# andimarafioti/faster-qwen3-tts

Measured on AMD Instinct MI355X. Metric: real-time factor (audio s / wall s), Qwen3-TTS-12Hz-0.6B voice-clone streaming chunk_size=8; p50 TTFA in ttfa_ms_p50, higher is better.
Workload: dtype bf16

## Files before the change

faster-qwen3-tts_amd/csrc/codec_kernels.cuh:

```cuda
#pragma once
#include "fq3_common.cuh"
#include "skinny_gemm.cuh"

namespace fq3 {

typedef __attribute__((ext_vector_type(8))) __bf16 bf16x8_t;
typedef __attribute__((ext_vector_type(4))) float f32x4_t;

constexpr int kMaxTaps = 8;
struct GemmArgs {
    const void* A; int lda; int M; int a_rows;
    int m_lo;
    int n_taps; int tap_off[kMaxTaps]; int Cin;
    const void* W; int N;
    const void* bias; int bias_mod;
    const void* scale;
    const void* res; int ldr;
    void* Y; int ldy;
    int act;
    const void* sn_a; const void* sn_ib; void* Y2;
    int act2;
    float* ws; long ws_floats; int ksplit;
    int n_seg; long a_seg, y_seg, r_seg;
    int glds_min_wgs;
    int big_pair;
    const void* Wp;
    const void* Wi;
    int no_skinny;
    int glds_cap8;
    int chain;
    int glds_waves;
    int xcd_map;
    int epi_legacy;
};

// ... 583 lines not shown
#pragma unroll
            for (int j = 0; j < TN; ++j) {
                const int r = wc * (BN / WCOLS) + j * 16 + fr;
                bfr[j] = *reinterpret_cast<const bf16x8_t*>(bs + r * BK + (((ks * 4 + fq) ^ ((r >> 1) & 7)) * 8));
            }
#pragma unroll
            for (int i = 0; i < TM; ++i)
#pragma unroll
                for (int j = 0; j < TN; ++j) {
                    if constexpr (DBG == 1) { acc[i][j][0] += (float)af[i][0] + (float)bfr[j][0]; }
                    else acc[i][j] = __builtin_amdgcn_mfma_f32_16x16x32_bf16(af[i], bfr[j], acc[i][j], 0, 0, 0);
                }
        }
        buf = buf + 1 == STAGES ? 0 : buf + 1;
    }
    constexpr int kParkFloats = STAGES * (BM + BN) * BK * 2 / 4;
    if (NT == 512 || epi_can_park(a)) {
        __syncthreads();
        gemm_epilogue_parked<TE, BM, BN, TM, TN, kParkFloats, WCOLS, NT>(a, acc, m0, n0, wr, wc, lane, reinterpret_cast<float*>(glds_smem));
    } else {
        if constexpr (NT == 256) gemm_epilogue<TE, BM, BN, TM, TN>(a, acc, m0, n0, wr, wc, lane);
    }
}

template <int BN, int STAGES, typename TE = bf16_t, int NT = 256, int BM = 128, int DBG = 0>
inline void glds_go(const GemmArgs& a, hipStream_t s) {
    const int rows = a.M - a.m_lo;
    const size_t shm = (size_t)STAGES * (BM + BN) * 64 * 2;
    constexpr auto kern = glds_gemm_kernel<BN, STAGES, TE, NT, BM, DBG>;
    (void)lds_limit_at_least<kern>(shm);
    hipLaunchKernelGGL(kern, dim3((a.N + BN - 1) / BN, (rows + BM - 1) / BM, a.n_seg > 1 ? a.n_seg : 1), dim3(NT), shm, s, a);
}

template <int NW, int CH, typename TE = bf16_t>
__global__ __launch_bounds__(NW * 64) void chain_gemm_kernel(GemmArgs a_in) {
    typedef bf16_t T;
    constexpr int BM = 32, BN = 32, TM = 2, TN = 2, LDP = BN + 4, NT = NW * 64;
    __shared__ __attribute__((aligned(16))) float park[BM * LDP];
    const GemmArgs a = gemm_segment<T, TE>(a_in, (int)blockIdx.z);
    const int tid = threadIdx.x, lane = tid & 63, fr = lane & 15, fq = lane >> 4;
    const int wave = __builtin_amdgcn_readfirstlane(tid >> 6);
    const int m0 = a.m_lo + blockIdx.y * BM, n0 = blockIdx.x * BN;
    const int K = a.n_taps * a.Cin, nsteps = K / 32, nchunks = (nsteps + CH - 1) / CH;
    const T* A = reinterpret_cast<const T*>(a.A);
    const T* zero = reinterpret_cast<const T*>(g_gemm_zero_page) + fq * 8;
    int am[TM];
#pragma unroll
    for (int i = 0; i < TM; ++i) { const int m = m0 + i * 16 + fr; am[i] = m < a.M ? m : -(1 << 28); }
    const T* wrow[TN];
#pragma unroll
    for (int j = 0; j < TN; ++j) {
        int n = n0 + j * 16 + fr;
        n = n < a.N ? n : a.N - 1;
        wrow[j] = reinterpret_cast<const T*>(a.W) + (size_t)n * K + fq * 8;
    }
    u32x4 ar[CH][TM], wr[CH][TN];
    auto load_chunk = [&](int c) {
#pragma unroll
        for (int s = 0; s < CH; ++s) {
            int t = c * CH + s;
            t = t < nsteps ? t : nsteps - 1;
            const int k0 = t * 32, tap = k0 / a.Cin, ci = k0 - tap * a.Cin;
            const int toff = a_in.tap_off[tap];
#pragma unroll
            for (int i = 0; i < TM; ++i) {
                const int r = am[i] + toff;
                const T* src = (r >= 0 && r < a.a_rows) ? A + (size_t)r * a.lda + ci + fq * 8 : zero;
                ar[s][i] = *reinterpret_cast<const u32x4*>(src);
            }
#pragma unroll
            for (int j = 0; j < TN; ++j) wr[s][j] = *reinterpret_cast<const u32x4*>(wrow[j] + k0);
        }
    };
    if (wave < nchunks) load_chunk(wave);
    for (int c = 0; c < nchunks; ++c) {
        if (wave == (c % NW)) {
            f32x4_t acc[TM][TN];
#pragma unroll
            for (int i = 0; i < TM; ++i)
#pragma unroll
                for (int j = 0; j < TN; ++j)
#pragma unroll
                    for (int r = 0; r < 4; ++r) acc[i][j][r] = c ? park[(i * 16 + fq * 4 + r) * LDP + j * 16 + fr] : 0.f;
#pragma unroll
            for (int s = 0; s < CH; ++s) {
                if (c * CH + s < nsteps) {
#pragma unroll
                    for (int i = 0; i < TM; ++i)
#pragma unroll
                        for (int j = 0; j < TN; ++j)
                            acc[i][j] = __builtin_amdgcn_mfma_f32_16x16x32_bf16(__builtin_bit_cast(bf16x8_t, ar[s][i]), __builtin_bit_cast(bf16x8_t, wr[s][j]), acc[i][j], 0, 0, 0);
                }
            }
#pragma unroll
            for (int i = 0; i < TM; ++i)
#pragma unroll
                for (int j = 0; j < TN; ++j)
#pragma unroll
                    for (int r = 0; r < 4; ++r) park[(i * 16 + fq * 4 + r) * LDP + j * 16 + fr] = acc[i][j][r];
            if (c + NW < nchunks) load_chunk(c + NW);
        }
        __builtin_amdgcn_s_waitcnt(0xc07f);
        __builtin_amdgcn_s_barrier();
    }
    const EpiQ e = epiq_of(a);
    const bool quads = epi_quads_ok(a);
    for (int q = tid; q < BM * (BN / 4); q += NT) {
        const int row = q / (BN / 4), c4 = (q - row * (BN / 4)) * 4;
        const int m = m0 + row, n = n0 + c4;
        if (m >= a.M || n >= a.N) continue;
        if (quads) epi_quad<TE>(e, *reinterpret_cast<const f32x4_t*>(park + row * LDP + c4), m, n);
        else for (int cc = 0; cc < 4 && n + cc < a.N; ++cc) epilogue_elem<TE>(a, park[row * LDP + c4 + cc], m, n + cc);
    }
}
template <int NW, int CH, typename TE = bf16_t>
inline void chain_go(const GemmArgs& a, hipStream_t s) {
    const int rows = a.M - a.m_lo;
    hipLaunchKernelGGL((chain_gemm_kernel<NW, CH, TE>), dim3((a.N + 31) / 32, (rows + 31) / 32, a.n_seg > 1 ? a.n_seg : 1), dim3(NW * 64), 0, s, a);
}
inline bool chain_ok(const GemmArgs& a) {
    return a.Cin % 32 == 0 && a.act != 2 && a.ksplit <= 1 && !a.epi_legacy && a.lda % 8 == 0;
}

constexpr int kBigBM = 256, kBigBN = 256, kBigBK = 32, kBigStages = 4;
constexpr int kGldsMinWgs = 150;
template <int ST, bool TR, int BN, typename TE = bf16_t, bool PAIR = false>
__global__ __launch_bounds__(512) void big_gemm_kernel(GemmArgs a_in, int tiles_x, int tiles_seg, int tiles_total) {
    typedef bf16_t T;
    static_assert(!TR || std::is_same<TE, bf16_t>::value, "the register-layout (TR) epilogue stores bf16");
    constexpr int BM = kBigBM, BK = kBigBK, TM = 8, TN = BN / 64, WN = BN / 4, NPB = BN / 128, CP = 2 + NPB;
    static_assert(ST == 4, "ring of four stages");
    static_assert(BN == 256 || BN == 128, "256- or 128-wide tiles");
    extern __shared__ __attribute__((aligned(128))) unsigned char big_smem[];
    T* As = reinterpret_cast<T*>(big_smem);
    T* Bs = As + ST * BM * BK;
    const int tid = threadIdx.x, lane = tid & 63, fr = lane & 15, fq = lane >> 4;
    const int wave = __builtin_amdgcn_readfirstlane(tid >> 6);
    const int orig = blockIdx.x, xcd = orig & 7, q = tiles_total >> 3, r8 = tiles_total & 7;
    const int tile_all = (xcd < r8 ? xcd * (q + 1) : r8 * (q + 1) + (xcd - r8) * q) + (orig >> 3);
    const int seg = tile_all / tiles_seg, tile = tile_all - seg * tiles_seg;
    const GemmArgs a = gemm_segment<T, TE>(a_in, seg);
    const int m0 = a.m_lo + (tile / tiles_x) * BM, n0 = (tile % tiles_x) * BN;
    const int wr = wave >> 2, wc = wave & 3;
    const int K = a.n_taps * a.Cin, nsteps = K / BK;
    const T* A = reinterpret_cast<const T*>(a.A);
    const T* W = reinterpret_cast<const T*>(a.W);
    const T* zero = reinterpret_cast<const T*>(g_gemm_zero_page);
    f32x4_t acc[TM][TN];
#pragma unroll
    for (int i = 0; i < TM; ++i)
#pragma unroll
        for (int j = 0; j < TN; ++j) acc[i][j] = f32x4_t{0.f, 0.f, 0.f, 0.f};
// ... 261 lines not shown
}

template <typename T>
__global__ __launch_bounds__(256) void splitk_reduce_kernel(GemmArgs a) {
    const int rows = a.M - a.m_lo;
    const size_t e = (size_t)blockIdx.x * 256 + threadIdx.x;
    if (e >= (size_t)rows * a.N) return;
    const int mm = (int)(e / a.N), n = (int)(e % a.N), m = a.m_lo + mm;
    float sum = 0.f;
    for (int z = 0; z < a.ksplit; ++z) sum += a.ws[(size_t)z * rows * a.N + e];
    const int ch = n % a.bias_mod;
    float v = DT<T>::rnd(sum + (a.bias ? DT<T>::ld(reinterpret_cast<const T*>(a.bias) + ch) : 0.f));
    if (a.act == 1) v = DT<T>::rnd(gelu_exact(v));
    if (a.act == 3) v = DT<T>::rnd(v / (1.0f + expf(-v)));
    if (a.scale) v = DT<T>::rnd(DT<T>::ld(reinterpret_cast<const T*>(a.scale) + n) * v);
    if (a.res) v = v + DT<T>::ld(reinterpret_cast<const T*>(a.res) + (size_t)m * a.ldr + n);
    v = DT<T>::rnd(v);
    if (a.Y) DT<T>::st(reinterpret_cast<T*>(a.Y) + (size_t)m * a.ldy + n, v);
    if (a.Y2) DT<T>::st(reinterpret_cast<T*>(a.Y2) + (size_t)m * a.ldy + n,
                        snake_apply<T>(v, DT<T>::ld(reinterpret_cast<const T*>(a.sn_a) + ch), DT<T>::ld(reinterpret_cast<const T*>(a.sn_ib) + ch)));
}

template <typename T, int BM, int BN, typename TE = T>
inline void gemm_go(const GemmArgs& a, hipStream_t s) {
    constexpr int PF = (BM + BN) > 160 ? 2 : ((BM + BN) > 128 ? 4 : 8);
    dim3 grid((a.N + BN - 1) / BN, (a.M - a.m_lo + BM - 1) / BM, a.n_seg > 1 ? a.n_seg : 1);
    hipLaunchKernelGGL((conv_gemm_kernel<T, BM, BN, PF, TE>), grid, dim3(256), 0, s, a);
}
inline bool skinny_ok(const GemmArgs& a) {
    return a.ws && !a.no_skinny && a.n_taps == 1 && a.tap_off[0] == 0 && a.m_lo == 0 && a.M <= kSkinnyMaxRows && a.a_rows >= a.M && a.act == 0 &&
           !a.bias && !a.scale && !a.Y2 && a.Y && skinny_k_ok(a.Cin) && a.N % 32 == 0 && a.lda % 8 == 0 && a.ldy % 4 == 0 && (!a.res || a.ldr % 4 == 0);
}
template <typename T, typename TE>
inline void gemm_launch_te(const GemmArgs& a, hipStream_t s) {
    const int rows = a.M - a.m_lo, nseg = a.n_seg > 1 ? a.n_seg : 1;
    if (rows <= 0) return;
    if constexpr (sizeof(T) == 4) { gemm_go<T, 64, 64>(a, s); return; }
    else {
        constexpr bool kPlainBf16 = std::is_same<TE, bf16_t>::value;
        auto wgs = [&](int bm, int bn) { return (long)((rows + bm - 1) / bm) * ((a.N + bn - 1) / bn) * nseg; };
        if constexpr (kPlainBf16) {
        if (nseg == 1 && skinny_ok(a)) {
            SkinnyArgs k{};
            k.X = reinterpret_cast<const bf16_t*>(a.A); k.ldx = a.lda; k.M = a.M; k.W = reinterpret_cast<const bf16_t*>(a.W); k.N = a.N;
            k.res = reinterpret_cast<const bf16_t*>(a.res); k.ldr = a.ldr; k.Y = reinterpret_cast<bf16_t*>(a.Y); k.ldy = a.ldy;
            k.Wp = reinterpret_cast<const bf16_t*>(a.Wp);
            if (a.res) skinny_launch<SK_RESIDUAL>(k, a.Cin, s); else skinny_launch<SK_STORE>(k, a.Cin, s);
            return;
        }
        if (nseg == 1 && a.ws && a.n_taps == 1 && a.act != 2 && wgs(64, 32) < 384 && a.Cin >= 1536) {
            int S = 0;
            for (int cand : {8, 6, 4, 3, 2})
                if (a.Cin % (cand * 32) == 0 && a.Cin / (cand * 32) >= 12 && wgs(64, 32) * cand <= 1024 &&
                    (long)cand * rows * a.N <= a.ws_floats) { S = cand; break; }
            if (S > 1) {
                GemmArgs b = a;
                b.ksplit = S;
                dim3 grid((a.N + 31) / 32, (rows + 63) / 64, S);
                hipLaunchKernelGGL((conv_gemm_kernel<T, 64, 32, 8>), grid, dim3(256), 0, s, b);
                hipLaunchKernelGGL((splitk_reduce_kernel<T>), dim3((unsigned)(((size_t)rows * a.N + 255) / 256)), dim3(256), 0, s, b);
                return;
            }
        }
        }
        const bool n64 = a.N % 64 == 0 || a.N >= 512;
        if (a.act != 2 && a.Cin % 32 == 0) {
            if (big_tiling_pays(rows, a.N, kBigBN, nseg)) { big_go<TE>(a, s); return; }
            if (rows >= 1024 && a.N % 128 == 0 && big_tiling_pays(rows, a.N, 128, nseg)) {
                const bool plain = a.act == 0 && !a.scale && !a.res && !a.Y2;
                if constexpr (kPlainBf16) { if (plain) { big_go_t<true, 128>(a, s); return; } }
                big_go_t<false, 128, TE>(a, s);
                return;
            }
        }
        const long t64 = wgs(128, 64);
        const bool glds_shape = a.N % 64 == 0 && a.Cin % 64 == 0;
        const bool parks = a.act != 2 && a.ksplit <= 1 && !a.epi_legacy && a.glds_waves >= 0;
        const long t32 = wgs(32, 32);
        if (a.chain >= 0 && chain_ok(a) && t32 <= 224 && (long)a.n_taps * a.Cin >= 512 && (long)a.n_taps * a.Cin <= 4096) { chain_go<8, 8, TE>(a, s); return; }
        const long cap8 = std::is_same<TE, bfs_t>::value ? (a.glds_cap8 > 0 ? a.glds_cap8 : (1L << 30)) : 512;
        if (glds_shape && parks && t64 <= cap8 && (long)a.n_taps * a.Cin >= 512) {
            const long ta = a.N % 128 == 0 ? wgs(64, 128) : 0, tb = wgs(64, 64);
            if (ta >= 140 && ta <= cap8) glds_go<128, 3, TE, 512, 64>(a, s);
            else if (tb <= 256) glds_go<64, 3, TE, 512, 64>(a, s);
            else if (t64 <= 256) glds_go<64, 3, TE, 512>(a, s);
            else glds_go<64, 2, TE, 512>(a, s);
        } else if (glds_shape && t64 >= (a.glds_min_wgs > 0 ? a.glds_min_wgs : kGldsMinWgs)) {
            glds_go<64, 2, TE>(a, s);
        } else if (n64 && wgs(128, 64) >= 512) gemm_go<T, 128, 64, TE>(a, s);
        else if (a.act != 2 && !n64 && a.N % 96 == 0 && wgs(128, 96) >= 256) gemm_go<T, 128, 96, TE>(a, s);
        else if (a.act != 2 && !n64 && wgs(128, 32) >= 256) gemm_go<T, 128, 32, TE>(a, s);
        else if (n64 && (wgs(64, 64) >= 256 || a.act == 2)) gemm_go<T, 64, 64, TE>(a, s);
        else if (a.act == 2) gemm_go<T, 64, 64, TE>(a, s);
        else gemm_go<T, 64, 32, TE>(a, s);
    }
}
template <typename T>
inline void gemm_launch(const GemmArgs& a, hipStream_t s) {
    if constexpr (std::is_same<T, bfs_t>::value) {
        GemmArgs b = a;
        b.lda = 2 * a.lda; b.Cin = 2 * a.Cin; b.a_seg = 2 * a.a_seg;
        b.ws = nullptr;
        gemm_launch_te<bf16_t, bfs_t>(b, s);
    } else gemm_launch_te<T, T>(a, s);
}

template <typename T> __global__ void silu_mul_kernel(const T* gu, T* y, int rows, int I);

template <typename T>
inline void gemm_swiglu_halves(const GemmArgs& a, void* y, hipStream_t s) {
    const int I = a.N / 2;
    if constexpr (sizeof(T) == 2) {
        if (skinny_ok(a) && !a.res && I % 8 == 0) {
            SkinnyArgs k{};
            k.X = reinterpret_cast<const bf16_t*>(a.A); k.ldx = a.lda; k.M = a.M; k.W = reinterpret_cast<const bf16_t*>(a.W); k.N = a.N;
            k.Y = reinterpret_cast<bf16_t*>(y); k.ldy = I;
            k.Wp = reinterpret_cast<const bf16_t*>(a.Wp);
            skinny_launch<SK_SWIGLU>(k, a.Cin, s);
            return;
        }
    }
    if constexpr (std::is_same<T, bf16_t>::value) {
        const int rows = a.M - a.m_lo;
        if (a.Wi && !a.res && !a.bias && !a.scale && a.n_taps == 1 && a.N % 512 == 0 && a.Cin % 32 == 0 && a.n_seg <= 1 && I % 4 == 0 &&
            big_tiling_pays(rows, a.N, kBigBN, 1)) {
            GemmArgs b = a;
            b.W = a.Wi; b.act = 2; b.Y = y; b.ldy = I;
            big_go_t<true, kBigBN>(b, s);
            return;
        }
    }
    gemm_launch<T>(a, s);
    hipLaunchKernelGGL((silu_mul_kernel<T>), dim3((unsigned)(((size_t)a.M * I + 255) / 256)), dim3(256), 0, s, (const T*)a.Y, (T*)y, a.M, I);
}

struct RvqArgs { const void* books[32]; int nq; int n_first; int dim; };
template <typename T>
__global__ void rvq_gather_kernel(RvqArgs a, const int64_t* codes, T* first, T* rest, int Tn, int row_lo) {
// ... 210 lines not shown
```

faster-qwen3-tts_amd/csrc/fq3_codec.hip:

```cpp
#define FQ3_SKINNY_EXTERN
#include "../../include/fq3hip.h"
#include "codec_kernels.cuh"

#include <algorithm>
#include <climits>
#include <cmath>
#include <functional>
#include <map>
#include <string>
#include <vector>

using namespace fq3;

extern "C" const char* fq3_last_error(void);
extern "C" void fq3_set_error_(const char* msg);
static int cfail(int code, const std::string& m) { fq3_set_error_(m.c_str()); return code; }
#define CHIP(x) do { hipError_t e_ = (x); if (e_ != hipSuccess) return cfail(FQ3_EHIP, std::string(#x) + ": " + hipGetErrorString(e_)); } while (0)

struct fq3_codec {
    fq3_codec_config cfg{};
    int esz = 2;
    std::map<std::string, const void*> w;
    std::map<std::string, int64_t> wn;
    void* buf[4] = {nullptr, nullptr, nullptr, nullptr};
    size_t buf_elems = 0;
    void* snake_consts = nullptr;
    std::map<std::string, std::pair<const void*, const void*>> snake;
    bool ready = false;
    int glds_cap8 = 0;
    int fuse_units = 1;
};

constexpr int kPrefixOutRows = 48;
struct fq3_codec_prefix {
    fq3_codec* owner = nullptr;
    int ref_len = 0, n_pre = 0, n_kv = 0, n_out = 0;
    void *pre = nullptr, *kv = nullptr, *out = nullptr;
};

static int64_t samples_for(const fq3_codec_config& c, int64_t T) {
    int64_t n = T;
    for (int i = 0; i < c.n_upsample; ++i) n *= c.upsampling_ratios[i];
    for (int i = 0; i < c.n_rates; ++i) n = (n - 1) * c.upsample_rates[i];
    return n > 0 ? n : 0;
}

extern "C" int64_t fq3_codec_num_samples(const fq3_codec* c, int T) { return c ? samples_for(c->cfg, T) : -1; }

static size_t elems_for(const fq3_codec_config& cfg, int64_t T) {
    int64_t rows = T, mx = T * std::max(std::max(cfg.latent_dim * 4, 3 * cfg.n_heads * cfg.head_dim), cfg.decoder_dim);
    mx = std::max(mx, 2 * T * (int64_t)cfg.rvq_dim);
    for (int i = 0; i < cfg.n_upsample; ++i) { rows *= cfg.upsampling_ratios[i]; mx = std::max(mx, rows * cfg.latent_dim * 4); }
    mx = std::max(mx, rows * cfg.decoder_dim);
    int ch = cfg.decoder_dim;
    for (int i = 0; i < cfg.n_rates; ++i) { rows = (rows - 1) * cfg.upsample_rates[i]; ch /= 2; mx = std::max(mx, rows * ch); }
    return (size_t)mx + 64;
}

extern "C" int fq3_codec_create(const fq3_codec_config* cfg, fq3_codec** out) {
    if (!cfg || !out) return cfail(FQ3_EINVAL, "null argument");
    if (cfg->dtype != FQ3_BF16 && cfg->dtype != FQ3_F32 && cfg->dtype != FQ3_BF16X2) return cfail(FQ3_EINVAL, "dtype");
    if (cfg->n_upsample < 0 || cfg->n_upsample > 4 || cfg->n_rates < 1 || cfg->n_rates > 8) return cfail(FQ3_EINVAL, "upsample lists");
    if (cfg->num_quantizers > 32) return cfail(FQ3_EUNSUPPORTED, "codec dims");
    if (cfg->head_dim != 32 && cfg->head_dim != 64 && cfg->head_dim != 128) return cfail(FQ3_EUNSUPPORTED, "codec head_dim must be 32, 64 or 128");
    if (cfg->sliding_window < 1 || cfg->sliding_window > 128) return cfail(FQ3_EUNSUPPORTED, "codec sliding_window must be in 1..128");
    auto m32 = [](int v) { return v % 32 == 0; };
    int ch = cfg->decoder_dim;
    bool ok = m32(cfg->rvq_dim) && m32(cfg->codebook_dim) && m32(cfg->latent_dim) && m32(cfg->hidden) && m32(cfg->inter) &&
              m32(cfg->n_heads * cfg->head_dim) && m32(ch);
    for (int i = 0; i < cfg->n_rates; ++i) { ch /= 2; ok = ok && m32(ch); }
    if (!ok) return cfail(FQ3_EUNSUPPORTED, "every channel count must be a multiple of 32 (MFMA K step)");
    fq3_codec* c = new fq3_codec();
    c->cfg = *cfg;
    c->esz = cfg->dtype == FQ3_BF16 ? 2 : 4;
    c->buf_elems = elems_for(*cfg, cfg->max_frames);
    for (int i = 0; i < 4; ++i) {
        hipError_t e = hipMalloc(&c->buf[i], c->buf_elems * c->esz);
        if (e != hipSuccess) { for (int j = 0; j < i; ++j) (void)hipFree(c->buf[j]); delete c; return cfail(FQ3_EHIP, "hipMalloc codec workspace"); }
    }
    *out = c;
    return FQ3_OK;
}

extern "C" int fq3_codec_destroy(fq3_codec* c) {
    if (!c) return FQ3_OK;
    (void)hipDeviceSynchronize();
    for (int i = 0; i < 4; ++i) if (c->buf[i]) (void)hipFree(c->buf[i]);
    if (c->snake_consts) (void)hipFree(c->snake_consts);
    delete c;
    return FQ3_OK;
}

extern "C" int fq3_codec_set_option(fq3_codec* c, const char* key, int value) {
    if (!c || !key) return cfail(FQ3_EINVAL, "null argument");
    if (std::string(key) == "glds_cap8") c->glds_cap8 = value;
    else if (std::string(key) == "fuse_units") c->fuse_units = value;
    else return cfail(FQ3_EINVAL, std::string("unknown codec option: ") + key);
    return FQ3_OK;
}

extern "C" int fq3_codec_bind(fq3_codec* c, const char* name, const void* ptr, int64_t numel) {
    if (!c || !name || !ptr) return cfail(FQ3_EINVAL, "null argument");
    c->w[name] = ptr; c->wn[name] = numel; c->ready = false;
    return FQ3_OK;
}

static int need(fq3_codec* c, const std::string& n, int64_t numel, const void** out) {
    auto it = c->w.find(n);
    if (it == c->w.end()) return cfail(FQ3_ESTATE, "codec weight not bound: " + n);
    if (numel > 0 && c->wn[n] != numel) return cfail(FQ3_EINVAL, "codec weight has wrong size: " + n + " (" + std::to_string(c->wn[n]) + " vs " + std::to_string(numel) + ")");
    if (out) *out = it->second;
    return 0;
}

static std::vector<std::pair<std::string, int>> snake_sites(const fq3_codec_config& g) {
    std::vector<std::pair<std::string, int>> v;
    int ch = g.decoder_dim;
    for (int i = 0; i < g.n_rates; ++i) {
        const std::string b = "decoder.decoder." + std::to_string(i + 1) + ".block.";
        v.push_back({b + "0.", ch});
        ch /= 2;
        for (int j = 2; j <= 4; ++j) { v.push_back({b + std::to_string(j) + ".act1.", ch}); v.push_back({b + std::to_string(j) + ".act2.", ch}); }
    }
    v.push_back({"decoder.decoder." + std::to_string(g.n_rates + 1) + ".", ch});
    return v;
}

extern "C" int fq3_codec_finalize(fq3_codec* c, void* stream) {
    if (!c) return cfail(FQ3_EINVAL, "null codec");
    const auto& g = c->cfg;
    const int QD = g.n_heads * g.head_dim;
    int r;
    for (int j = 0; j < g.num_quantizers; ++j) {
        const bool first = j < g.num_semantic;
        const std::string n = std::string("decoder.quantizer.") + (first ? "rvq_first" : "rvq_rest") + ".vq.layers." +
                              std::to_string(first ? j : j - g.num_semantic) + "._codebook.embedding";
        if ((r = need(c, n, (int64_t)g.codebook_size * g.rvq_dim, nullptr))) return r;
    }
    if ((r = need(c, "decoder.pre_conv.conv.weight", (int64_t)g.latent_dim * 3 * g.codebook_dim, nullptr))) return r;
    if ((r = need(c, "decoder.pre_transformer.layers.0.self_attn.qkv.weight", (int64_t)3 * QD * g.hidden, nullptr))) return r;
    if ((r = need(c, "decoder.pre_transformer.layers.0.mlp.gate_up.weight", (int64_t)2 * g.inter * g.hidden, nullptr))) return r;
    if (g.inter % 16) return cfail(FQ3_EUNSUPPORTED, "codec intermediate size must be a multiple of 16");
    if ((r = need(c, "rope.cos", (int64_t)g.max_frames * (g.head_dim / 2), nullptr))) return r;
    if ((r = need(c, "rope.sin", (int64_t)g.max_frames * (g.head_dim / 2), nullptr))) return r;
    const auto sites = snake_sites(g);
    size_t total = 0;
    for (auto& s : sites) total += 2 * (size_t)s.second;
    if (c->snake_consts) { (void)hipFree(c->snake_consts); c->snake_consts = nullptr; }
    CHIP(hipMalloc(&c->snake_consts, total * c->esz));
    size_t off = 0;
    hipStream_t st = (hipStream_t)stream;
    for (auto& s : sites) {
        const void *al = nullptr, *be = nullptr;
        if ((r = need(c, s.first + "alpha", s.second, &al)) || (r = need(c, s.first + "beta", s.second, &be))) return r;
        char* base = (char*)c->snake_consts + off * c->esz;
        void* pa = base; void* pib = base + (size_t)s.second * c->esz;
        if (g.dtype == FQ3_BF16) hipLaunchKernelGGL((snake_consts_kernel<bf16_t>), dim3((s.second + 255) / 256), dim3(256), 0, st, (const bf16_t*)al, (const bf16_t*)be, (bf16_t*)pa, (bf16_t*)pib, s.second);
        else if (g.dtype == FQ3_BF16X2) hipLaunchKernelGGL((snake_consts_kernel<bfs_t>), dim3((s.second + 255) / 256), dim3(256), 0, st, (const bfs_t*)al, (const bfs_t*)be, (bfs_t*)pa, (bfs_t*)pib, s.second);
        else hipLaunchKernelGGL((snake_consts_kernel<float>), dim3((s.second + 255) / 256), dim3(256), 0, st, (const float*)al, (const float*)be, (float*)pa, (float*)pib, s.second);
        c->snake[s.first] = {pa, pib};
        off += 2 * (size_t)s.second;
    }
    CHIP(hipStreamSynchronize(st));
    c->ready = true;
    return FQ3_OK;
}

namespace {
enum { DEP_SAME = 0, DEP_BACK = 1, DEP_DIV = 2, DEP_ALL = 3 };
struct Dep { int t; int kind; int p; };
struct Op {
    int out = -1, out2 = -1;
    std::vector<Dep> in;
    int unit = 1;
    std::function<void(int lo)> run;
};
struct Plan {
    std::vector<Op> ops;
    int n_tensors = 0;
    int tensor() { return n_tensors++; }
    void add(Op&& o) { ops.push_back(std::move(o)); }
};
}

template <typename T>
static GemmArgs lin(const void* A, int M, int Kc, const void* W, int N, const void* bias, void* Y) {
    GemmArgs a{}; a.A = A; a.lda = Kc; a.M = M; a.a_rows = M; a.n_taps = 1; a.tap_off[0] = 0; a.Cin = Kc; a.W = W; a.N = N;
    a.bias = bias; a.bias_mod = N; a.Y = Y; a.ldy = N; return a;
}
static GemmArgs conv(const void* A, int rows, int Cin, const void* W, int Cout, const void* bias, void* Y, int k, int dil) {
    GemmArgs a{}; a.A = A; a.lda = Cin; a.M = rows; a.a_rows = rows; a.n_taps = k; a.Cin = Cin; a.W = W; a.N = Cout;
    for (int i = 0; i < k; ++i) a.tap_off[i] = -(k - 1 - i) * dil;
    a.bias = bias; a.bias_mod = Cout; a.Y = Y; a.ldy = Cout; return a;
}

static GemmArgs segmented(GemmArgs a, int NS) {
    a.n_seg = NS; a.a_seg = (long)a.a_rows * a.lda; a.y_seg = (long)a.M * a.ldy; a.r_seg = (long)a.M * a.ldr;
    return a;
}

constexpr int kPrefixTooShort = -1000;
template <typename T>
static int decode_t(fq3_codec* c, const int64_t* codes, int NS, int Tn, int64_t first_sample, float* pcm, hipStream_t s,
                    const fq3_codec_prefix* const* pfx = nullptr, fq3_codec_prefix* cap = nullptr) {
    const auto& g = c->cfg;
    int err = 0;
    const int f0 = pfx ? pfx[0]->ref_len : 0;
    PrefixSrc src_pre{}, src_kv{}, src_out{};
    if (pfx) for (int u = 0; u < NS; ++u) { src_pre.p[u] = pfx[u]->pre; src_kv.p[u] = pfx[u]->kv; src_out.p[u] = pfx[u]->out; }
    auto W = [&](const std::string& n) -> const void* { const void* p = nullptr; if (!err) err = need(c, n, 0, &p); return p; };
    auto SN = [&](const std::string& prefix) -> std::pair<const void*, const void*> {
        auto it = c->snake.find(prefix);
        if (it == c->snake.end()) { if (!err) err = cfail(FQ3_ESTATE, "snake constants missing: " + prefix); return {nullptr, nullptr}; }
        return it->second;
    };
    T* B0 = (T*)c->buf[0]; T* B1 = (T*)c->buf[1]; T* B2 = (T*)c->buf[2]; T* B3 = (T*)c->buf[3];
    const std::string D = "decoder.";
    auto el = [&](size_t n) { return dim3((unsigned)((n + 255) / 256), (unsigned)NS); };
    const dim3 rows4((Tn - f0 + 3) / 4, NS);
    Plan P;
    auto gemm_op = [&](GemmArgs a, int out, int out2, std::vector<Dep> in, int unit = 1) {
        Op o; o.out = out; o.out2 = out2; o.in = std::move(in); o.unit = unit;
        a = segmented(a, NS);
        a.glds_cap8 = c->glds_cap8;
        o.run = [a, s](int lo) mutable { a.m_lo = lo; gemm_launch<T>(a, s); };
        P.add(std::move(o));
    };
    auto G = [&](GemmArgs a) { a.m_lo = f0; a.glds_cap8 = c->glds_cap8; gemm_launch<T>(segmented(a, NS), s); };
    auto put_rows = [&](const PrefixSrc& src, size_t src_off, int src_ld, T* dst, int dst_ld, int dst_col0, int n_rows, int n_cols) {
        if (n_rows <= 0) return;
        constexpr int EPC = 16 / (int)sizeof(T);
        hipLaunchKernelGGL((prefix_rows_kernel<T>), dim3((n_rows * (n_cols / EPC) + 255) / 256, NS), dim3(256), 0, s, src, src_off, src_ld, dst,
                           (size_t)Tn * dst_ld, dst_ld, f0 - n_rows, dst_col0, n_rows, n_cols);
    };
    auto keep_rows = [&](void* dst, size_t dst_off, int dst_ld, const T* src, int src_ld, int src_col0, int n_rows, int n_cols) {
        if (n_rows <= 0) return;
        (void)hipMemcpy2DAsync((T*)dst + dst_off, (size_t)dst_ld * sizeof(T), src + (size_t)(Tn - n_rows) * src_ld + src_col0, (size_t)src_ld * sizeof(T),
                               (size_t)n_cols * sizeof(T), n_rows, hipMemcpyDeviceToDevice, s);
    };

    RvqArgs ra{}; ra.nq = g.num_quantizers; ra.n_first = g.num_semantic; ra.dim = g.rvq_dim;
    for (int j = 0; j < g.num_quantizers; ++j) {
        const bool first = j < g.num_semantic;
        ra.books[j] = W(D + "quantizer." + (first ? "rvq_first" : "rvq_rest") + ".vq.layers." +
                        std::to_string(first ? j : j - g.num_semantic) + "._codebook.embedding");
    }
    if (err) return err;
    const int t_front = P.tensor();
    {
        Op o; o.out = t_front;
        const void* w_first = W(D + "quantizer.rvq_first.output_proj.weight");
        const void* w_rest = W(D + "quantizer.rvq_rest.output_proj.weight");
        const void* w_pre = W(D + "pre_conv.conv.weight"); const void* b_pre = W(D + "pre_conv.conv.bias");
        const std::string TR = D + "pre_transformer.";
        const void* w_in = W(TR + "input_proj.weight"); const void* b_in = W(TR + "input_proj.bias");
        const int QD = g.n_heads * g.head_dim;
        const float* cosT = (const float*)W("rope.cos"); const float* sinT = (const float*)W("rope.sin");
        struct LayerW { const void *ln1, *qkv, *o, *ls1, *ln2, *gu, *down, *ls2; };
        std::vector<LayerW> LW(g.n_layers);
        for (int i = 0; i < g.n_layers; ++i) {
            const std::string L = TR + "layers." + std::to_string(i) + ".";
            LW[i] = {W(L + "input_layernorm.weight"), W(L + "self_attn.qkv.weight"), W(L + "self_attn.o_proj.weight"),
                     W(L + "self_attn_layer_scale.scale"), W(L + "post_attention_layernorm.weight"), W(L + "mlp.gate_up.weight"),
                     W(L + "mlp.down_proj.weight"), W(L + "mlp_layer_scale.scale")};
        }
        const void* w_norm = W(TR + "norm.weight");
        const void* w_out = W(TR + "output_proj.weight"); const void* b_out = W(TR + "output_proj.bias");
        if (err) return err;
        o.run = [=](int) {
            T* qf = B1; T* qr = B1 + (size_t)NS * Tn * g.rvq_dim;
            hipLaunchKernelGGL((rvq_gather_kernel<T>), dim3(Tn - f0, NS), dim3(256), 0, s, ra, codes, qf, qr, Tn, f0);
            G(lin<T>(qf, Tn, g.rvq_dim, w_first, g.codebook_dim, nullptr, B0));
            { GemmArgs a = lin<T>(qr, Tn, g.rvq_dim, w_rest, g.codebook_dim, nullptr, B0); a.res = B0; a.ldr = g.codebook_dim; G(a); }
            if (pfx) put_rows(src_pre, 0, g.codebook_dim, B0, g.codebook_dim, 0, pfx[0]->n_pre, g.codebook_dim);
            if (cap) keep_rows(cap->pre, 0, g.codebook_dim, B0, g.codebook_dim, 0, cap->n_pre, g.codebook_dim);
            G(conv(B0, Tn, g.codebook_dim, w_pre, g.latent_dim, b_pre, B1, 3, 1));
            G(lin<T>(B1, Tn, g.latent_dim, w_in, g.hidden, b_in, B0));
            for (int i = 0; i < g.n_layers; ++i) {
                const LayerW& w = LW[i];
                hipLaunchKernelGGL((rmsnorm_rows_kernel<T>), rows4, dim3(256), 0, s, (const T*)B0, (const T*)w.ln1, B1, f0, Tn, g.hidden, g.rms_eps);
                G(lin<T>(B1, Tn, g.hidden, w.qkv, 3 * QD, nullptr, B2));
                hipLaunchKernelGGL((rope_rows_kernel<T>), el((size_t)(Tn - f0) * 2 * g.n_heads * (g.head_dim / 2)), dim3(256), 0, s, B2, cosT, sinT, Tn, QD, g.head_dim, f0);
                if (pfx) put_rows(src_kv, (size_t)i * pfx[0]->n_kv * 2 * QD, 2 * QD, B2, 3 * QD, QD, pfx[0]->n_kv, 2 * QD);
                if (cap) keep_rows(cap->kv, (size_t)i * cap->n_kv * 2 * QD, 2 * QD, B2, 3 * QD, QD, cap->n_kv, 2 * QD);
                const dim3 ag((Tn - f0 + 3) / 4, g.n_heads, NS);
                const float sc = 1.0f / sqrtf((float)g.head_dim);
                if (g.head_dim == 32) hipLaunchKernelGGL((swa_attn_kernel<T, 32>), ag, dim3(256), 0, s, (const T*)B2, B1, Tn, g.n_heads, g.sliding_window, sc, f0);
                else if (g.head_dim == 64) hipLaunchKernelGGL((swa_attn_kernel<T, 64>), ag, dim3(256), 0, s, (const T*)B2, B1, Tn, g.n_heads, g.sliding_window, sc, f0);
                else hipLaunchKernelGGL((swa_attn_kernel<T, 128>), ag, dim3(256), 0, s, (const T*)B2, B1, Tn, g.n_heads, g.sliding_window, sc, f0);
                { GemmArgs a = lin<T>(B1, Tn, QD, w.o, g.hidden, nullptr, B0); a.scale = w.ls1; a.res = B0; a.ldr = g.hidden; G(a); }
                hipLaunchKernelGGL((rmsnorm_rows_kernel<T>), rows4, dim3(256), 0, s, (const T*)B0, (const T*)w.ln2, B1, f0, Tn, g.hidden, g.rms_eps);
                { GemmArgs a = lin<T>(B1, Tn, g.hidden, w.gu, 2 * g.inter, nullptr, B2); a.act = 2; a.ldy = g.inter; G(a); }
                { GemmArgs a = lin<T>(B2, Tn, g.inter, w.down, g.hidden, nullptr, B0); a.scale = w.ls2; a.res = B0; a.ldr = g.hidden; G(a); }
            }
            hipLaunchKernelGGL((rmsnorm_rows_kernel<T>), rows4, dim3(256), 0, s, (const T*)B0, (const T*)w_norm, B1, f0, Tn, g.hidden, g.rms_eps);
            G(lin<T>(B1, Tn, g.hidden, w_out, g.latent_dim, b_out, B0));
            if (pfx) put_rows(src_out, 0, g.latent_dim, B0, g.latent_dim, 0, pfx[0]->n_out, g.latent_dim);
            if (cap) keep_rows(cap->out, 0, g.latent_dim, B0, g.latent_dim, 0, cap->n_out, g.latent_dim);
        };
        if (cap) { o.run(0); return err; }
        P.add(std::move(o));
    }
    const int kFrontSame = pfx ? DEP_SAME : DEP_ALL, kFrontBack = pfx ? DEP_BACK : DEP_ALL;
    int rows = Tn;
    const int Lc = g.latent_dim;
    int t_h = t_front;
    for (int i = 0; i < g.n_upsample && !err; ++i) {
        const int f = g.upsampling_ratios[i];
        const std::string U = D + "upsample." + std::to_string(i) + ".";
        const int t_up = P.tensor(), t_dw = P.tensor(), t_ln = P.tensor(), t_pw = P.tensor(), t_o = P.tensor();
        { GemmArgs a = lin<T>(B0, rows, Lc, W(U + "0.conv.weight"), f * Lc, W(U + "0.conv.bias"), B1); a.bias_mod = Lc;
          gemm_op(a, t_up, -1, {{t_h, t_h == t_front ? kFrontSame : DEP_SAME, 0}}, f); }
        rows *= f;
        {
            const int R = rows;
            const T* dw = (const T*)W(U + "1.dwconv.conv.weight"); const T* db = (const T*)W(U + "1.dwconv.conv.bias");
            Op o; o.out = t_dw; o.in = {{t_up, DEP_BACK, 6}};
            o.run = [=](int lo) { if (lo < R) hipLaunchKernelGGL((dwconv7_kernel<T>), el((size_t)(R - lo) * Lc), dim3(256), 0, s, (const T*)B1, dw, db, B2, lo, R, Lc); };
            P.add(std::move(o));
            const T* nw = (const T*)W(U + "1.norm.weight"); const T* nb = (const T*)W(U + "1.norm.bias");
            Op o2; o2.out = t_ln; o2.in = {{t_dw, DEP_SAME, 0}};
            o2.run = [=](int lo) { if (lo < R) hipLaunchKernelGGL((layernorm_rows_kernel<T>), dim3((R - lo + 3) / 4, NS), dim3(256), 0, s, (const T*)B2, nw, nb, B3, lo, R, Lc, 1e-6f); };
            P.add(std::move(o2));
        }
        { GemmArgs a = lin<T>(B3, rows, Lc, W(U + "1.pwconv1.weight"), 4 * Lc, W(U + "1.pwconv1.bias"), B2); a.act = 1;
          gemm_op(a, t_pw, -1, {{t_ln, DEP_SAME, 0}}); }
        { GemmArgs a = lin<T>(B2, rows, 4 * Lc, W(U + "1.pwconv2.weight"), Lc, W(U + "1.pwconv2.bias"), B0);
          a.scale = W(U + "1.gamma"); a.res = B1; a.ldr = Lc;
          gemm_op(a, t_o, -1, {{t_pw, DEP_SAME, 0}, {t_up, DEP_SAME, 0}}); }
// ... 212 lines not shown
```

Before: 38.92.

## Pre-pack codec GEMM weights into MFMA-fragment images for the chain kernel

At finalize, weights for eligible codec GEMM sites are repacked into a fragment-ordered image so each lane's 16-byte weight load in the chain GEMM kernel is contiguous across lanes, instead of strided by row K. The chain kernel gains a PACKED variant that reads from this image, and the dispatcher uses it when an image serves the weight, also widening the tile limit for the chain path. This costs extra device memory for duplicated weights and a one-time pack at load, and may route more shapes to the chain kernel than before.

```diff
diff --git a/faster-qwen3-tts_amd/csrc/chain_pack_map.h b/faster-qwen3-tts_amd/csrc/chain_pack_map.h
--- /dev/null
+++ b/faster-qwen3-tts_amd/csrc/chain_pack_map.h
@@ -0,0 +1,22 @@
+#pragma once
+#include <cstddef>
+#include <cstdint>
+
+#if defined(__HIPCC__) || defined(__CUDACC__)
+#define FQ3_HD __host__ __device__
+#else
+#define FQ3_HD
+#endif
+
+namespace fq3 {
+
+constexpr int kChainSlotBytes = 1024;
+
+FQ3_HD constexpr int chain_img_blocks(int N) { return 2 * ((N + 31) / 32); }
+FQ3_HD constexpr int chain_img_slots(int K) { return K / 32; }
+FQ3_HD constexpr size_t chain_img_bytes(int N, int K) { return (size_t)chain_img_blocks(N) * chain_img_slots(K) * kChainSlotBytes; }
+FQ3_HD constexpr size_t chain_img_frag(int nb, int t, int lane, int nslots) { return (((size_t)nb * nslots + t) * 64 + lane) * 16; }
+FQ3_HD constexpr int chain_img_row(int nb, int lane, int N) { return nb * 16 + (lane & 15) < N ? nb * 16 + (lane & 15) : N - 1; }
+FQ3_HD constexpr int chain_img_col(int t, int lane, int e) { return 32 * t + 8 * (lane >> 4) + e; }
+
+}
diff --git a/faster-qwen3-tts_amd/csrc/codec_kernels.cuh b/faster-qwen3-tts_amd/csrc/codec_kernels.cuh
--- a/faster-qwen3-tts_amd/csrc/codec_kernels.cuh
+++ b/faster-qwen3-tts_amd/csrc/codec_kernels.cuh
@@ -1,6 +1,7 @@
 #pragma once
 #include "fq3_common.cuh"
 #include "skinny_gemm.cuh"
+#include "chain_pack_map.h"
 
 namespace fq3 {
 
@@ -650,8 +651,8 @@
     hipLaunchKernelGGL(kern, dim3((a.N + BN - 1) / BN, (rows + BM - 1) / BM, a.n_seg > 1 ? a.n_seg : 1), dim3(NT), shm, s, a);
 }
 
-template <int NW, int CH, typename TE = bf16_t>
-__global__ __launch_bounds__(NW * 64) void chain_gemm_kernel(GemmArgs a_in) {
+template <int NW, int CH, typename TE = bf16_t, bool PACKED = false>
+__global__ __launch_bounds__(NW * 64) void chain_gemm_kernel(GemmArgs a_in, const void* img) {
     typedef bf16_t T;
     constexpr int BM = 32, BN = 32, TM = 2, TN = 2, LDP = BN + 4, NT = NW * 64;
     __shared__ __attribute__((aligned(16))) float park[BM * LDP];
@@ -666,11 +667,16 @@
 #pragma unroll
     for (int i = 0; i < TM; ++i) { const int m = m0 + i * 16 + fr; am[i] = m < a.M ? m : -(1 << 28); }
     const T* wrow[TN];
+    const unsigned char* wimg[TN];
 #pragma unroll
     for (int j = 0; j < TN; ++j) {
-        int n = n0 + j * 16 + fr;
-        n = n < a.N ? n : a.N - 1;
-        wrow[j] = reinterpret_cast<const T*>(a.W) + (size_t)n * K + fq * 8;
+        if constexpr (!PACKED) {
+            int n = n0 + j * 16 + fr;
+            n = n < a.N ? n : a.N - 1;
+            wrow[j] = reinterpret_cast<const T*>(a.W) + (size_t)n * K + fq * 8;
+        } else {
+            wimg[j] = reinterpret_cast<const unsigned char*>(img) + chain_img_frag(n0 / 16 + j, 0, lane, nsteps);
+        }
     }
     u32x4 ar[CH][TM], wr[CH][TN];
     auto load_chunk = [&](int c) {
@@ -687,7 +693,10 @@
                 ar[s][i] = *reinterpret_cast<const u32x4*>(src);
             }
 #pragma unroll
-            for (int j = 0; j < TN; ++j) wr[s][j] = *reinterpret_cast<const u32x4*>(wrow[j] + k0);
+            for (int j = 0; j < TN; ++j) {
+                if constexpr (PACKED) wr[s][j] = *reinterpret_cast<const u32x4*>(wimg[j] + (size_t)t * kChainSlotBytes);
+                else wr[s][j] = *reinterpret_cast<const u32x4*>(wrow[j] + k0);
+            }
         }
     };
     if (wave < nchunks) load_chunk(wave);
@@ -734,8 +743,56 @@
 template <int NW, int CH, typename TE = bf16_t>
 inline void chain_go(const GemmArgs& a, hipStream_t s) {
     const int rows = a.M - a.m_lo;
-    hipLaunchKernelGGL((chain_gemm_kernel<NW, CH, TE>), dim3((a.N + 31) / 32, (rows + 31) / 32, a.n_seg > 1 ? a.n_seg : 1), dim3(NW * 64), 0, s, a);
-}
+    hipLaunchKernelGGL((chain_gemm_kernel<NW, CH, TE>), dim3((a.N + 31) / 32, (rows + 31) / 32, a.n_seg > 1 ? a.n_seg : 1), dim3(NW * 64), 0, s, a, (const void*)nullptr);
+}
+
+template <int DUMMY = 0>
+__global__ void chain_pack_kernel(const unsigned short* W, u32x4* img, int N, int K) {
+    const int nslots = chain_img_slots(K);
+    const size_t f = (size_t)blockIdx.x * blockDim.x + threadIdx.x, total = (size_t)chain_img_blocks(N) * nslots * 64;
+    if (f >= total) return;
+    const int lane = (int)(f & 63), t = (int)((f >> 6) % nslots), nb = (int)((f >> 6) / nslots);
+    const unsigned short* row = W + (size_t)chain_img_row(nb, lane, N) * K;
+    uint32_t d[4];
+#pragma unroll
+    for (int e = 0; e < 8; e += 2)
+        d[e / 2] = (uint32_t)row[chain_img_col(t, lane, e)] | (uint32_t)row[chain_img_col(t, lane, e + 1)] << 16;
+    img[chain_img_frag(nb, t, lane, nslots) / 16] = u32x4{d[0], d[1], d[2], d[3]};
+}
+inline void chain_pack_launch(const void* W, void* img, int N, int K, hipStream_t s) {
+    const size_t frags = chain_img_bytes(N, K) / 16;
+    hipLaunchKernelGGL(chain_pack_kernel<0>, dim3((unsigned)((frags + 255) / 256)), dim3(256), 0, s, reinterpret_cast<const unsigned short*>(W),
+                       reinterpret_cast<u32x4*>(img), N, K);
+}
+struct ChainImage { void* img = nullptr; const void* W = nullptr; int N = 0, K = 0; };
+inline bool chain_shape_ok(int N, int K) { return N > 0 && K > 0 && K % 32 == 0; }
+inline void chain_image_at(ChainImage& ci, void* mem, const void* W, int N, int K, hipStream_t s) {
+    chain_pack_launch(W, mem, N, K, s);
+    ci.img = mem; ci.W = W; ci.N = N; ci.K = K;
+}
+typedef hipError_t (*chain_alloc_fn)(void**, size_t);
+inline bool chain_image_build(ChainImage& ci, const void* W, int N, int K, hipStream_t s, chain_alloc_fn alloc = nullptr) {
+    ci = ChainImage{};
+    if (!W || !chain_shape_ok(N, K)) return false;
+    const size_t bytes = chain_img_bytes(N, K);
+    void* p = nullptr;
+    const hipError_t e = alloc ? alloc(&p, bytes) : hipMalloc(&p, bytes);
+    if (e != hipSuccess || !p) { (void)hipGetLastError(); return false; }
+    chain_image_at(ci, p, W, N, K, s);
+    return true;
+}
+inline void chain_image_free(ChainImage& ci) { if (ci.img) (void)hipFree(ci.img); ci = ChainImage{}; }
+inline bool chain_image_serves(const ChainImage* ci, const GemmArgs& a) {
+    return ci && ci->img && ci->W == a.W && ci->N == a.N && ci->K == a.n_taps * a.Cin && chain_shape_ok(ci->N, ci->K);
+}
+template <int NW, int CH, typename TE = bf16_t>
+inline void chain_go_img(const GemmArgs& a, const ChainImage* ci, hipStream_t s) {
+    if (!chain_image_serves(ci, a)) { chain_go<NW, CH, TE>(a, s); return; }
+    const int rows = a.M - a.m_lo;
+    const dim3 grid((a.N + 31) / 32, (rows + 31) / 32, a.n_seg > 1 ? a.n_seg : 1);
+    hipLaunchKernelGGL((chain_gemm_kernel<NW, CH, TE, true>), grid, dim3(NW * 64), 0, s, a, (const void*)ci->img);
+}
+constexpr long kChainImgMaxTiles = 256, kChainImgMaxK = 4096;
 inline bool chain_ok(const GemmArgs& a) {
     return a.Cin % 32 == 0 && a.act != 2 && a.ksplit <= 1 && !a.epi_legacy && a.lda % 8 == 0;
 }
@@ -1063,7 +1120,7 @@
            !a.bias && !a.scale && !a.Y2 && a.Y && skinny_k_ok(a.Cin) && a.N % 32 == 0 && a.lda % 8 == 0 && a.ldy % 4 == 0 && (!a.res || a.ldr % 4 == 0);
 }
 template <typename T, typename TE>
-inline void gemm_launch_te(const GemmArgs& a, hipStream_t s) {
+inline void gemm_launch_te(const GemmArgs& a, hipStream_t s, const ChainImage* ci = nullptr) {
     const int rows = a.M - a.m_lo, nseg = a.n_seg > 1 ? a.n_seg : 1;
     if (rows <= 0) return;
     if constexpr (sizeof(T) == 4) { gemm_go<T, 64, 64>(a, s); return; }
@@ -1108,7 +1165,11 @@
         const bool glds_shape = a.N % 64 == 0 && a.Cin % 64 == 0;
         const bool parks = a.act != 2 && a.ksplit <= 1 && !a.epi_legacy && a.glds_waves >= 0;
         const long t32 = wgs(32, 32);
-        if (a.chain >= 0 && chain_ok(a) && t32 <= 224 && (long)a.n_taps * a.Cin >= 512 && (long)a.n_taps * a.Cin <= 4096) { chain_go<8, 8, TE>(a, s); return; }
+        const long kk = (long)a.n_taps * a.Cin;
+        if (a.chain >= 0 && chain_ok(a) && kk >= 512) {
+            if (chain_image_serves(ci, a) && t32 <= kChainImgMaxTiles && kk <= kChainImgMaxK) { chain_go_img<8, 8, TE>(a, ci, s); return; }
+            if (t32 <= 224 && kk <= 4096) { chain_go<8, 8, TE>(a, s); return; }
+        }
         const long cap8 = std::is_same<TE, bfs_t>::value ? (a.glds_cap8 > 0 ? a.glds_cap8 : (1L << 30)) : 512;
         if (glds_shape && parks && t64 <= cap8 && (long)a.n_taps * a.Cin >= 512) {
             const long ta = a.N % 128 == 0 ? wgs(64, 128) : 0, tb = wgs(64, 64);
@@ -1127,14 +1188,16 @@
     }
 }
 template <typename T>
-inline void gemm_launch(const GemmArgs& a, hipStream_t s) {
+inline void gemm_launch_img(const GemmArgs& a, hipStream_t s, const ChainImage* ci) {
     if constexpr (std::is_same<T, bfs_t>::value) {
         GemmArgs b = a;
         b.lda = 2 * a.lda; b.Cin = 2 * a.Cin; b.a_seg = 2 * a.a_seg;
         b.ws = nullptr;
-        gemm_launch_te<bf16_t, bfs_t>(b, s);
-    } else gemm_launch_te<T, T>(a, s);
-}
+        gemm_launch_te<bf16_t, bfs_t>(b, s, ci);
+    } else gemm_launch_te<T, T>(a, s, ci);
+}
+template <typename T>
+inline void gemm_launch(const GemmArgs& a, hipStream_t s) { gemm_launch_img<T>(a, s, nullptr); }
 
 template <typename T> __global__ void silu_mul_kernel(const T* gu, T* y, int rows, int I);
 
diff --git a/faster-qwen3-tts_amd/csrc/fq3_codec.hip b/faster-qwen3-tts_amd/csrc/fq3_codec.hip
--- a/faster-qwen3-tts_amd/csrc/fq3_codec.hip
+++ b/faster-qwen3-tts_amd/csrc/fq3_codec.hip
@@ -8,6 +8,7 @@
 #include <functional>
 #include <map>
 #include <string>
+#include <tuple>
 #include <vector>
 
 using namespace fq3;
@@ -27,6 +28,9 @@
     void* snake_consts = nullptr;
     std::map<std::string, std::pair<const void*, const void*>> snake;
     bool ready = false;
+    std::map<const void*, ChainImage> chain_img;
+    void* chain_mem = nullptr;
+    int chain_packed = 1;
     int glds_cap8 = 0;
     int fuse_units = 1;
 };
@@ -87,6 +91,7 @@
     (void)hipDeviceSynchronize();
     for (int i = 0; i < 4; ++i) if (c->buf[i]) (void)hipFree(c->buf[i]);
     if (c->snake_consts) (void)hipFree(c->snake_consts);
+    if (c->chain_mem) (void)hipFree(c->chain_mem);
     delete c;
     return FQ3_OK;
 }
@@ -94,6 +99,7 @@
 extern "C" int fq3_codec_set_option(fq3_codec* c, const char* key, int value) {
     if (!c || !key) return cfail(FQ3_EINVAL, "null argument");
     if (std::string(key) == "glds_cap8") c->glds_cap8 = value;
+    else if (std::string(key) == "chain_packed") c->chain_packed = value;
     else if (std::string(key) == "fuse_units") c->fuse_units = value;
     else return cfail(FQ3_EINVAL, std::string("unknown codec option: ") + key);
     return FQ3_OK;
@@ -124,6 +130,66 @@
     }
     v.push_back({"decoder.decoder." + std::to_string(g.n_rates + 1) + ".", ch});
     return v;
+}
+
+static std::vector<std::tuple<std::string, int, int>> gemm_sites(const fq3_codec_config& g) {
+    std::vector<std::tuple<std::string, int, int>> v;
+    const std::string D = "decoder.", TR = D + "pre_transformer.", DD = D + "decoder.";
+    const int QD = g.n_heads * g.head_dim, Lc = g.latent_dim;
+    v.emplace_back(D + "quantizer.rvq_first.output_proj.weight", g.codebook_dim, g.rvq_dim);
+    v.emplace_back(D + "quantizer.rvq_rest.output_proj.weight", g.codebook_dim, g.rvq_dim);
+    v.emplace_back(D + "pre_conv.conv.weight", Lc, 3 * g.codebook_dim);
+    v.emplace_back(TR + "input_proj.weight", g.hidden, Lc);
+    for (int i = 0; i < g.n_layers; ++i) {
+        const std::string L = TR + "layers." + std::to_string(i) + ".";
+        v.emplace_back(L + "self_attn.qkv.weight", 3 * QD, g.hidden);
+        v.emplace_back(L + "self_attn.o_proj.weight", g.hidden, QD);
+        v.emplace_back(L + "mlp.down_proj.weight", g.hidden, g.inter);
+    }
+    v.emplace_back(TR + "output_proj.weight", Lc, g.hidden);
+    for (int i = 0; i < g.n_upsample; ++i) {
+        const std::string U = D + "upsample." + std::to_string(i) + ".";
+        v.emplace_back(U + "0.conv.weight", g.upsampling_ratios[i] * Lc, Lc);
+        v.emplace_back(U + "1.pwconv1.weight", 4 * Lc, Lc);
+        v.emplace_back(U + "1.pwconv2.weight", Lc, 4 * Lc);
+    }
+    int ch = g.decoder_dim;
+    v.emplace_back(DD + "0.conv.weight", ch, 7 * Lc);
+    for (int i = 0; i < g.n_rates; ++i) {
+        const std::string Bk = DD + std::to_string(i + 1) + ".block.";
+        v.emplace_back(Bk + "1.conv.weight", g.upsample_rates[i] * (ch / 2), 2 * ch);
+        ch /= 2;
+        for (int j = 2; j <= 4; ++j) {
+            v.emplace_back(Bk + std::to_string(j) + ".conv1.conv.weight", ch, 7 * ch);
+            v.emplace_back(Bk + std::to_string(j) + ".conv2.conv.weight", ch, ch);
+        }
+    }
+    return v;
+}
+
+static void build_chain_images(fq3_codec* c, hipStream_t st) {
+    c->chain_img.clear();
+    if (c->chain_mem) { (void)hipFree(c->chain_mem); c->chain_mem = nullptr; }
+    if (c->cfg.dtype == FQ3_F32) return;
+    const bool x2 = c->cfg.dtype == FQ3_BF16X2;
+    struct Served { const void* W; int N, K; size_t off; };
+    std::vector<Served> served;
+    size_t total = 0;
+    for (auto& site : gemm_sites(c->cfg)) {
+        const std::string& name = std::get<0>(site);
+        const int N = std::get<1>(site), K = (x2 ? 2 : 1) * std::get<2>(site);
+        auto it = c->w.find(name);
+        if (it == c->w.end() || c->wn[name] != (int64_t)N * std::get<2>(site)) continue;
+        if (K < 512 || K > kChainImgMaxK || (N + 31) / 32 > kChainImgMaxTiles || !chain_shape_ok(N, K)) continue;
+        bool seen = false;
+        for (auto& sv : served) seen = seen || sv.W == it->second;
+        if (seen) continue;
+        served.push_back({it->second, N, K, total});
+        total += (chain_img_bytes(N, K) + 4095) & ~(size_t)4095;
+    }
+    if (!total) return;
+    if (hipMalloc(&c->chain_mem, total) != hipSuccess) { (void)hipGetLastError(); c->chain_mem = nullptr; return; }
+    for (auto& sv : served) chain_image_at(c->chain_img[sv.W], (char*)c->chain_mem + sv.off, sv.W, sv.N, sv.K, st);
 }
 
 extern "C" int fq3_codec_finalize(fq3_codec* c, void* stream) {
@@ -161,6 +227,7 @@
         c->snake[s.first] = {pa, pib};
         off += 2 * (size_t)s.second;
     }
+    build_chain_images(c, st);
     CHIP(hipStreamSynchronize(st));
     c->ready = true;
     return FQ3_OK;
@@ -219,14 +286,20 @@
     auto el = [&](size_t n) { return dim3((unsigned)((n + 255) / 256), (unsigned)NS); };
     const dim3 rows4((Tn - f0 + 3) / 4, NS);
     Plan P;
+    auto IMG = [&](const void* w) -> const ChainImage* {
+        if (!c->chain_packed) return nullptr;
+        auto it = c->chain_img.find(w);
+        return it == c->chain_img.end() ? nullptr : &it->second;
+    };
     auto gemm_op = [&](GemmArgs a, int out, int out2, std::vector<Dep> in, int unit = 1) {
         Op o; o.out = out; o.out2 = out2; o.in = std::move(in); o.unit = unit;
         a = segmented(a, NS);
         a.glds_cap8 = c->glds_cap8;
-        o.run = [a, s](int lo) mutable { a.m_lo = lo; gemm_launch<T>(a, s); };
+        const ChainImage* ci = IMG(a.W);
+        o.run = [a, s, ci](int lo) mutable { a.m_lo = lo; gemm_launch_img<T>(a, s, ci); };
         P.add(std::move(o));
     };
-    auto G = [&](GemmArgs a) { a.m_lo = f0; a.glds_cap8 = c->glds_cap8; gemm_launch<T>(segmented(a, NS), s); };
+    auto G = [&](GemmArgs a, const ChainImage* ci) { a.m_lo = f0; a.glds_cap8 = c->glds_cap8; gemm_launch_img<T>(segmented(a, NS), s, ci); };
     auto put_rows = [&](const PrefixSrc& src, size_t src_off, int src_ld, T* dst, int dst_ld, int dst_col0, int n_rows, int n_cols) {
         if (n_rows <= 0) return;
         constexpr int EPC = 16 / (int)sizeof(T);
@@ -256,30 +329,32 @@
         const void* w_in = W(TR + "input_proj.weight"); const void* b_in = W(TR + "input_proj.bias");
         const int QD = g.n_heads * g.head_dim;
         const float* cosT = (const float*)W("rope.cos"); const float* sinT = (const float*)W("rope.sin");
-        struct LayerW { const void *ln1, *qkv, *o, *ls1, *ln2, *gu, *down, *ls2; };
+        struct LayerW { const void *ln1, *qkv, *o, *ls1, *ln2, *gu, *down, *ls2; const ChainImage *i_qkv, *i_o, *i_down; };
         std::vector<LayerW> LW(g.n_layers);
         for (int i = 0; i < g.n_layers; ++i) {
             const std::string L = TR + "layers." + std::to_string(i) + ".";
             LW[i] = {W(L + "input_layernorm.weight"), W(L + "self_attn.qkv.weight"), W(L + "self_attn.o_proj.weight"),
                      W(L + "self_attn_layer_scale.scale"), W(L + "post_attention_layernorm.weight"), W(L + "mlp.gate_up.weight"),
-                     W(L + "mlp.down_proj.weight"), W(L + "mlp_layer_scale.scale")};
+                     W(L + "mlp.down_proj.weight"), W(L + "mlp_layer_scale.scale"), nullptr, nullptr, nullptr};
+            LW[i].i_qkv = IMG(LW[i].qkv); LW[i].i_o = IMG(LW[i].o); LW[i].i_down = IMG(LW[i].down);
         }
         const void* w_norm = W(TR + "norm.weight");
         const void* w_out = W(TR + "output_proj.weight"); const void* b_out = W(TR + "output_proj.bias");
+        const ChainImage *i_first = IMG(w_first), *i_rest = IMG(w_rest), *i_pre = IMG(w_pre), *i_in = IMG(w_in), *i_out = IMG(w_out);
         if (err) return err;
         o.run = [=](int) {
             T* qf = B1; T* qr = B1 + (size_t)NS * Tn * g.rvq_dim;
             hipLaunchKernelGGL((rvq_gather_kernel<T>), dim3(Tn - f0, NS), dim3(256), 0, s, ra, codes, qf, qr, Tn, f0);
-            G(lin<T>(qf, Tn, g.rvq_dim, w_first, g.codebook_dim, nullptr, B0));
-            { GemmArgs a = lin<T>(qr, Tn, g.rvq_dim, w_rest, g.codebook_dim, nullptr, B0); a.res = B0; a.ldr = g.codebook_dim; G(a); }
+            G(lin<T>(qf, Tn, g.rvq_dim, w_first, g.codebook_dim, nullptr, B0), i_first);
+            { GemmArgs a = lin<T>(qr, Tn, g.rvq_dim, w_rest, g.codebook_dim, nullptr, B0); a.res = B0; a.ldr = g.codebook_dim; G(a, i_rest); }
             if (pfx) put_rows(src_pre, 0, g.codebook_dim, B0, g.codebook_dim, 0, pfx[0]->n_pre, g.codebook_dim);
             if (cap) keep_rows(cap->pre, 0, g.codebook_dim, B0, g.codebook_dim, 0, cap->n_pre, g.codebook_dim);
-            G(conv(B0, Tn, g.codebook_dim, w_pre, g.latent_dim, b_pre, B1, 3, 1));
-            G(lin<T>(B1, Tn, g.latent_dim, w_in, g.hidden, b_in, B0));
+            G(conv(B0, Tn, g.codebook_dim, w_pre, g.latent_dim, b_pre, B1, 3, 1), i_pre);
+            G(lin<T>(B1, Tn, g.latent_dim, w_in, g.hidden, b_in, B0), i_in);
             for (int i = 0; i < g.n_layers; ++i) {
                 const LayerW& w = LW[i];
                 hipLaunchKernelGGL((rmsnorm_rows_kernel<T>), rows4, dim3(256), 0, s, (const T*)B0, (const T*)w.ln1, B1, f0, Tn, g.hidden, g.rms_eps);
-                G(lin<T>(B1, Tn, g.hidden, w.qkv, 3 * QD, nullptr, B2));
+                G(lin<T>(B1, Tn, g.hidden, w.qkv, 3 * QD, nullptr, B2), w.i_qkv);
                 hipLaunchKernelGGL((rope_rows_kernel<T>), el((size_t)(Tn - f0) * 2 * g.n_heads * (g.head_dim / 2)), dim3(256), 0, s, B2, cosT, sinT, Tn, QD, g.head_dim, f0);
                 if (pfx) put_rows(src_kv, (size_t)i * pfx[0]->n_kv * 2 * QD, 2 * QD, B2, 3 * QD, QD, pfx[0]->n_kv, 2 * QD);
                 if (cap) keep_rows(cap->kv, (size_t)i * cap->n_kv * 2 * QD, 2 * QD, B2, 3 * QD, QD, cap->n_kv, 2 * QD);
@@ -288,13 +363,13 @@
                 if (g.head_dim == 32) hipLaunchKernelGGL((swa_attn_kernel<T, 32>), ag, dim3(256), 0, s, (const T*)B2, B1, Tn, g.n_heads, g.sliding_window, sc, f0);
                 else if (g.head_dim == 64) hipLaunchKernelGGL((swa_attn_kernel<T, 64>), ag, dim3(256), 0, s, (const T*)B2, B1, Tn, g.n_heads, g.sliding_window, sc, f0);
                 else hipLaunchKernelGGL((swa_attn_kernel<T, 128>), ag, dim3(256), 0, s, (const T*)B2, B1, Tn, g.n_heads, g.sliding_window, sc, f0);
-                { GemmArgs a = lin<T>(B1, Tn, QD, w.o, g.hidden, nullptr, B0); a.scale = w.ls1; a.res = B0; a.ldr = g.hidden; G(a); }
+                { GemmArgs a = lin<T>(B1, Tn, QD, w.o, g.hidden, nullptr, B0); a.scale = w.ls1; a.res = B0; a.ldr = g.hidden; G(a, w.i_o); }
                 hipLaunchKernelGGL((rmsnorm_rows_kernel<T>), rows4, dim3(256), 0, s, (const T*)B0, (const T*)w.ln2, B1, f0, Tn, g.hidden, g.rms_eps);
-                { GemmArgs a = lin<T>(B1, Tn, g.hidden, w.gu, 2 * g.inter, nullptr, B2); a.act = 2; a.ldy = g.inter; G(a); }
-                { GemmArgs a = lin<T>(B2, Tn, g.inter, w.down, g.hidden, nullptr, B0); a.scale = w.ls2; a.res = B0; a.ldr = g.hidden; G(a); }
+                { GemmArgs a = lin<T>(B1, Tn, g.hidden, w.gu, 2 * g.inter, nullptr, B2); a.act = 2; a.ldy = g.inter; G(a, nullptr); }
+                { GemmArgs a = lin<T>(B2, Tn, g.inter, w.down, g.hidden, nullptr, B0); a.scale = w.ls2; a.res = B0; a.ldr = g.hidden; G(a, w.i_down); }
             }
             hipLaunchKernelGGL((rmsnorm_rows_kernel<T>), rows4, dim3(256), 0, s, (const T*)B0, (const T*)w_norm, B1, f0, Tn, g.hidden, g.rms_eps);
-            G(lin<T>(B1, Tn, g.hidden, w_out, g.latent_dim, b_out, B0));
+            G(lin<T>(B1, Tn, g.hidden, w_out, g.latent_dim, b_out, B0), i_out);
             if (pfx) put_rows(src_out, 0, g.latent_dim, B0, g.latent_dim, 0, pfx[0]->n_out, g.latent_dim);
             if (cap) keep_rows(cap->out, 0, g.latent_dim, B0, g.latent_dim, 0, cap->n_out, g.latent_dim);
         };
```

New measurement: 38.91, median of 4. No clear change (-0.0%).
